# sd-james/gym-treasure-game

Hardware: AMD Instinct MI355X
Metric: env-steps/sec (whole node) at 1M batched envs, 1/2/4/8 MI355X; bit-exact vs CPU (higher is better)
Workload: dtype int32+f64

## Files before the change

gym-treasure-game_amd/_lib.py:

```python
import ctypes
import os

HERE = os.path.dirname(os.path.abspath(__file__))
LIB_PATH = os.environ.get("TG_LIB_PATH") or os.path.join(HERE, "libtg_amd.so")

TG_OK = 0
TG_STEP_AUTORESET = 1
TG_POLICY_UNIFORM = 0
TG_POLICY_MASKED = 1
TG_MODE_DIRECT = 0
TG_MODE_COMPACT = 1
TG_MODE_FLOW = 2
TG_ERR_TICKCAP = 1 << 24
TG_ERR_BAG = 1 << 25
TG_ERR_ACTION = 1 << 26
TG_ERR_NEARINT = 1 << 27
TG_ERR_RENDER = 1 << 28
TG_ERR_WINDOW = 1 << 29
TG_ERR_FLOW = 1 << 30
TG_SPR_COUNT = 24
TG_FRAME_RGB = 3
TG_FRAME_GRAY = 1
TG_ACT_RELU = 0
TG_ACT_TANH = 1
# ... 16 lines not shown

class TgError(RuntimeError):
    pass


class Episode(ctypes.Structure):
    _fields_ = [("env", ctypes.c_int64), ("ret", ctypes.c_int32), ("len", ctypes.c_int32)]


class PyState(ctypes.Structure):
    _fields_ = [("mt", ctypes.c_uint32 * 624), ("index", ctypes.c_uint32),
                ("has_gauss", ctypes.c_uint32), ("gauss_next", ctypes.c_double)]


class Stats(ctypes.Structure):
    _fields_ = [("steps", ctypes.c_int64), ("valid_steps", ctypes.c_int64),
                ("ticks", ctypes.c_int64), ("draws", ctypes.c_int64),
                ("episodes", ctypes.c_int64), ("episodes_dropped", ctypes.c_int64),
                ("launches", ctypes.c_int64),
                ("kernel_ms", ctypes.c_double), ("regens", ctypes.c_int64),
                ("wave_ticks", ctypes.c_int64), ("timed_launches", ctypes.c_int64),
                ("run_ms", ctypes.c_double), ("regen_ms", ctypes.c_double),
                ("regen_timed", ctypes.c_int64), ("regen_launches", ctypes.c_int64),
                ("classify_ms", ctypes.c_double)]

    def as_dict(self):
        return {k: getattr(self, k) for k, _ in self._fields_}


_lib = None


def load():
    global _lib
    if _lib is not None:
        return _lib
    if not os.path.exists(LIB_PATH):
        raise TgError("libtg_amd.so is not built (%s); run __graft_entry__.build() or "
                      "python -m gym_treasure_game_amd.build" % LIB_PATH)
    L = ctypes.CDLL(LIB_PATH)
    P, i32, i64, u32, u64 = (ctypes.c_void_p, ctypes.c_int32, ctypes.c_int64, ctypes.c_uint32,
                             ctypes.c_uint64)
    sig = {
        "tg_create": (i32, [ctypes.POINTER(P), i64, u64, i64, i32, ctypes.c_char_p,
                            ctypes.c_char_p, ctypes.c_char_p]),
        "tg_destroy": (None, [P]),
        "tg_num_envs": (i64, [P]),
# ... 55 lines not shown
```

gym-treasure-game_amd/csrc/tg_amd.hip:

```cpp
#include <hip/hip_runtime.h>

#include <algorithm>
#include <chrono>
#include <cstdio>
#include <cstdlib>
#include <cstring>
#include <mutex>
#include <string>
#include <type_traits>
#include <vector>

#include "../../include/tg_amd.h"
#include "tg_dev.h"
#include "tg_flow.h"
#include "tg_kernels.h"
#include "tg_py1.h"

namespace tg {
thread_local std::string g_err;
}

namespace {

int grid_for(int64_t n) { return (int)((n + BLOCK - 1) / BLOCK); }
int run_grid_for(int64_t n) { return grid_for(n) + (NLIST * 64 + BLOCK - 1) / BLOCK; }
int stat_slots(int64_t n) { return run_grid_for(n); }

#define ALLOC(ptr, bytes)                               \
  if (hipMalloc((void**)&(ptr), (bytes)) != hipSuccess) \
    return fail(TG_E_NOMEM, "hipMalloc %zu B for " #ptr, (size_t)(bytes))

constexpr int KST_MAX = 512;
constexpr int64_t KST_KSLOTS = (int64_t)KST_MAX * 3 * KST_SLOTS;
unsigned long long* kst_step(tg_batch* h, int k, int kernel) {
  return h->kst + ((size_t)k * 2 + kernel) * KST_STRIDE * KST_SLOTS;
}
unsigned long long* kst_regen(tg_batch* h, int k) {
  return h->kst + ((size_t)KST_MAX * 2 + k) * KST_STRIDE * KST_SLOTS;
}
int kst_reset(tg_batch* h) {
  if (!h->kst && hipMalloc((void**)&h->kst, sizeof(unsigned long long) * KST_STRIDE * KST_KSLOTS) !=
                     hipSuccess)
    return fail(TG_E_NOMEM, "timing records");
  hipLaunchKernelGGL(k_kst_init, dim3((unsigned)((KST_KSLOTS + BLOCK - 1) / BLOCK)), dim3(BLOCK), 0, 0,
                     h->kst, KST_KSLOTS);
  HIP_TRY(hipGetLastError());
  HIP_TRY(hipDeviceSynchronize());
  h->kst_steps = 0;
// ... 33 lines not shown
  if (!h->timing_every || (h->timing_calls++ % (uint64_t)h->timing_every) != 0) return TG_OK;
  if (h->kst_steps >= KST_MAX)
    if (const int rc = flush_timing(h)) return rc;
  ks0 = kst_step(h, h->kst_steps, 0);
  ks1 = kst_step(h, h->kst_steps, 1);
  ++h->kst_steps;
  h->kst_k.push_back(k);
  return TG_OK;
}

int alloc_ctx(StepCtx& c, int64_t off, int64_t n) {
  c.off = off;
  c.n = n;
  ALLOC(c.stats, sizeof(unsigned long long) * ST_COUNT * (size_t)stat_slots(n));
  c.shard_cap = (int64_t)((grid_for(n) + WSHARDS - 1) / WSHARDS) * BLOCK;
  ALLOC(c.wl, sizeof(int32_t) * NSEG * (size_t)c.shard_cap);
  ALLOC(c.wst4, sizeof(uint4) * NSEG * (size_t)c.shard_cap);
  ALLOC(c.wang, sizeof(double2) * NSEG * (size_t)c.shard_cap);
  ALLOC(c.wep, sizeof(int2) * NSEG * (size_t)c.shard_cap);
  ALLOC(c.wctr, sizeof(int32_t) * 2 * NCTR * CTR_STRIDE);
  c.rcap = (int64_t)((grid_for(n) + SHARDS - 1) / SHARDS) * BLOCK * REGEN_STEPS;
  ALLOC(c.refill, sizeof(uint32_t) * SHARDS * (size_t)c.rcap);
  ALLOC(c.regen_ctr, sizeof(int32_t) * 2 * RCTR_N * CTR_STRIDE);
  HIP_TRY(hipMemset(c.stats, 0, sizeof(unsigned long long) * ST_COUNT * (size_t)stat_slots(n)));
  HIP_TRY(hipMemset(c.wctr, 0, sizeof(int32_t) * 2 * NCTR * CTR_STRIDE));
  HIP_TRY(hipMemset(c.regen_ctr, 0, sizeof(int32_t) * 2 * RCTR_N * CTR_STRIDE));
  return TG_OK;
}
void free_ctx(StepCtx& c) {
  void* bufs[] = {c.stats, c.wl, c.wst4, c.wang, c.wep, c.wctr, c.refill, c.regen_ctr};
  for (void* b : bufs)
    if (b) (void)hipFree(b);
  if (c.ev) (void)hipEventDestroy(c.ev);
  if (c.st) (void)hipStreamDestroy(c.st);
  c = StepCtx{};
}
Soa soa_of(const tg_batch* h, const StepCtx& c) {
  return Soa{h->S.st4 + c.off, h->S.ang + c.off, h->S.ep + c.off, h->S.mt + c.off * (int64_t)MT_STORE,
             h->S.mc + c.off * (int64_t)MT_CODES};
}
int launch_regen(tg_batch* h, StepCtx& c, hipStream_t st) {
  if (!c.rpend) return TG_OK;
  unsigned long long* ks = nullptr;
  if (h->timing_every && &c == &h->main) {
    if (h->kst_regens >= KST_MAX) {
      const int rc = flush_timing(h);
      if (rc) return rc;
    }
    ks = kst_regen(h, h->kst_regens++);
  }
  if (!h->regen_per_cu) {
    int nb = 0;
    HIP_TRY(hipOccupancyMaxActiveBlocksPerMultiprocessor(&nb, reinterpret_cast<const void*>(k_regen),
// ... 42 lines not shown
    io.valid += c.off;
    io.done += c.off;
    if (io.final_obs) io.final_obs += c.off * 9;
  }
  const bool fo = io.final_obs != nullptr;
  unsigned long long *ks0 = nullptr, *ks1 = nullptr;
  if (&c == &h->main || &c == h->grp.data())
    if (const int rc = timing_begin(h, ks0, ks1)) return rc;
  const EpQueue q{h->eps, h->eps_count, h->eps_cap};
  const dim3 grid(grid_for(c.n)), block(BLOCK);
  const Soa S = soa_of(h, c);
  const int64_t g0 = h->g0 + c.off;
  if (h->mode == TG_MODE_DIRECT) {
    const auto kern = step_inst(ar, fo, io.policy,
                                [](auto AR, auto FO, auto POL) { return &k_step<AR, FO, POL>; });
    hipLaunchKernelGGL(kern, grid, block, 0, st, S, c.n, h->L, h->grid, io, q, g0, c.stats, h->err,
                       ks1);
  } else {
    int32_t* const cur = c.wctr + (c.parity ? NCTR * CTR_STRIDE : 0);
    int32_t* const nxt = c.wctr + (c.parity ? 0 : NCTR * CTR_STRIDE);
    c.parity ^= 1;
    const Work w{c.wl,     c.wst4, c.wang, c.wep, cur, nxt, c.refill,
                 c.regen_ctr + (c.regen_parity * RCTR_N + RCTR_LIST) * CTR_STRIDE, c.rcap,
                 c.shard_cap};
    const auto kc = step_inst(ar, fo, io.policy,
                              [](auto AR, auto FO, auto POL) { return &k_classify<AR, FO, POL>; });
    const auto kr = step_inst(ar, fo, -1, [](auto AR, auto FO, auto) { return &k_run<AR, FO>; });
    hipLaunchKernelGGL(kc, grid, block, 0, st, S, c.n, h->L, h->grid, io, q, w, g0, c.stats, h->err,
                       ks0);
    HIP_TRY(hipGetLastError());
    if (mid) HIP_TRY(hipEventRecord(mid, st));
    hipLaunchKernelGGL(kr, dim3(run_grid_for(c.n) * (BLOCK / RUN_BLOCK)), dim3(RUN_BLOCK), 0, st, S,
                       c.n, h->L, h->grid, io, q, w,
                       g0, c.stats, h->err, ks1);
  }
  HIP_TRY(hipGetLastError());
  if (h->mode != TG_MODE_DIRECT && ++c.rpend == REGEN_STEPS) return launch_regen(h, c, st);
  return TG_OK;
}

int rollout_prep(tg_batch* h, const char* who, int32_t steps, bool selector_ok, const double* obs,
                 const int32_t* reward, const uint8_t* valid, const uint8_t* done) {
  if (steps < 0 || !reward || !valid || !done || !selector_ok)
    return fail(TG_E_INVAL, "%s: bad arguments", who);
  if (!obs && !h->obs_scratch)
    if (hipMalloc((void**)&h->obs_scratch, sizeof(double) * 9 * (size_t)h->n) != hipSuccess)
      return fail(TG_E_NOMEM, "%s: obs scratch", who);
// ... 1015 lines not shown
  HIP_TRY(hipDeviceSynchronize());
  int rc = flush_timing(h);
  if (rc) return rc;
  unsigned long long s[ST_COUNT] = {};
  std::vector<StepCtx*> ctxs{&h->main};
  for (auto& c : h->grp) ctxs.push_back(&c);
  for (StepCtx* c : ctxs) {
    const size_t nb = (size_t)stat_slots(c->n);
    std::vector<unsigned long long> part(nb * ST_COUNT);
    HIP_TRY(hipMemcpy(part.data(), c->stats, sizeof(unsigned long long) * part.size(),
                      hipMemcpyDeviceToHost));
    for (size_t b = 0; b < nb; ++b)
      for (int k = 0; k < ST_COUNT; ++k) s[k] += part[b * ST_COUNT + k];
  }
  out->steps = (int64_t)s[ST_STEPS];
  out->valid_steps = (int64_t)s[ST_VALID];
  out->ticks = (int64_t)s[ST_TICKS];
  out->draws = (int64_t)s[ST_DRAWS];
  out->episodes = (int64_t)s[ST_EPISODES];
  out->episodes_dropped = (int64_t)s[ST_EP_OVERFLOW];
  out->launches = out->steps / (h->n ? h->n : 1);
  out->kernel_ms = h->kernel_ms_done;
  out->regens = (int64_t)s[ST_REGENS] * MT_HALF_GENS;
  out->wave_ticks = (int64_t)s[ST_WTICKS];
  out->timed_launches = h->timed_launches;
  out->run_ms = h->run_ms_done;
  out->regen_ms = h->regen_ms_done;
  out->regen_timed = h->regen_timed;
  out->regen_launches = h->regen_launches;
  out->classify_ms = h->classify_ms_done;
  return TG_OK;
}

int tg_stats_reset(tg_batch* h) {
  BIND(h);
  HIP_TRY(hipDeviceSynchronize());
  HIP_TRY(hipMemset(h->main.stats, 0, sizeof(unsigned long long) * ST_COUNT * (size_t)stat_slots(h->n)));
  for (auto& c : h->grp)
    HIP_TRY(hipMemset(c.stats, 0, sizeof(unsigned long long) * ST_COUNT * (size_t)stat_slots(c.n)));
  if (h->kst) {
    const int rc = kst_reset(h);
    if (rc) return rc;
  }
  h->kernel_ms_done = 0.0;
  h->run_ms_done = 0.0;
  h->classify_ms_done = 0.0;
// ... 65 lines not shown
```

gym-treasure-game_amd/csrc/tg_batch.h:

```cpp
#pragma once
#include <hip/hip_runtime.h>

#include <cstdarg>
#include <cstdio>
#include <string>
#include <vector>

#include "../../include/tg_amd.h"
#include "tg_core.h"

namespace tg {

extern thread_local std::string g_err;
inline int fail(int code, const char* fmt, ...) __attribute__((format(printf, 2, 3)));
inline int fail(int code, const char* fmt, ...) {
  char buf[512];
  va_list ap;
  va_start(ap, fmt);
  vsnprintf(buf, sizeof buf, fmt, ap);
  va_end(ap);
  g_err = buf;
  return code;
}
#define HIP_TRY(expr)                                                                    \
// ... 35 lines not shown
  uint32_t pad2[2];
  uint64_t t_seen, t_end;
  uint32_t ticks;
  uint32_t pad3[7];
  uint64_t phase[5];
  uint64_t pad4[3];
};
static_assert(sizeof(SrvBox) == 192, "SrvBox: three 64-B lines");

struct RenderState;
void render_free(RenderState* rs);

struct StepCtx {
  int64_t off = 0, n = 0;
  unsigned long long* stats = nullptr;
  int32_t* wl = nullptr;
  uint4* wst4 = nullptr;
  double2* wang = nullptr;
  int2* wep = nullptr;
  int32_t* wctr = nullptr;
  uint32_t* refill = nullptr;
  int64_t rcap = 0;
  int64_t shard_cap = 0;
  int parity = 0;
  int rpend = 0;
  int32_t* regen_ctr = nullptr;
  int regen_parity = 0;
  hipStream_t st = nullptr;
  hipEvent_t ev = nullptr;
};

}

struct tg_batch {
  int device = 0;
  int64_t n = 0;
  int64_t g0 = 0;
  uint64_t seed0 = 0;
  tg::Level L{};
  uint32_t* grid = nullptr;
  uint32_t* genrand = nullptr;
  uint32_t* gotab = nullptr;
  uint32_t* masks = nullptr;
  double* obs_q = nullptr;
  int cus = 0;
  tg::Soa S{};
// ... 98 lines not shown
```

gym-treasure-game_amd/csrc/tg_dev.h:

```cpp
#pragma once
#include <hip/hip_runtime.h>

#include "../../include/tg_amd.h"
#include "tg_core.h"
#include "tg_level.h"
#include "tg_batch.h"
#include "tg_twist.h"
#include "tg_run_diag.h"

using namespace tg;

namespace {

constexpr int BLOCK = 256;
#ifndef TG_RUN_BLOCK
#define TG_RUN_BLOCK 256
#endif
constexpr int RUN_BLOCK = TG_RUN_BLOCK;
static_assert(RUN_BLOCK % 64 == 0 && BLOCK % RUN_BLOCK == 0, "whole waves, whole k_classify blocks");
constexpr int PRIO_SLOW = 3;

__device__ __forceinline__ void unpack_st4(const uint4 s, Env& e) {
  e.px = (int)(int16_t)(s.x & 0xFFFFu);
  e.py = (int)(int16_t)(s.x >> 16);
// ... 26 lines not shown
TG_HD int grid_words(int W, int H) { return ((W + 2 * PAD) * (H + 2 * PAD) + 3) / 4; }
template <int NT = BLOCK>
__device__ __forceinline__ void stage_cells(uint32_t* lgrid, uint32_t* ltrig,
                                            const uint32_t* __restrict__ grid, const Level& L,
                                            uint32_t* masks = nullptr) {
  const int nwords = grid_words(L.W, L.H);
  for (int i = threadIdx.x; i < nwords; i += NT) lgrid[i] = grid[i];
  if (threadIdx.x < 12) ltrig[threadIdx.x] = L.trig[threadIdx.x >> 1][threadIdx.x & 1];
  if (masks && L.masks)
    for (int i = threadIdx.x; i < mk_words(L.W, L.H); i += NT) masks[i] = L.masks[i];
  __syncthreads();
}
struct LevelView {
  const uint32_t* trig;
  Map m;
  uint8_t* win;
};
__device__ __forceinline__ LevelView level_in_lds(const uint32_t* __restrict__ grid, const Level& L) {
  __shared__ LdsLevel lv;
  stage_cells(lv.grid, lv.trig, grid, L);
  return {lv.trig, Map{reinterpret_cast<const uint8_t*>(lv.grid), L.W, L.H}, nullptr};
}
template <int NT, int WAVE_BYTES>
__device__ __forceinline__ LevelView run_level_in_lds(const uint32_t* __restrict__ grid, const Level& L) {
  __shared__ uint4 run_lds[((NT / 64) * WAVE_BYTES + MAX_CELLS + 4 * MK_MAX_WORDS) / 16];
  __shared__ uint32_t ltrig[12];
  uint8_t* const win = reinterpret_cast<uint8_t*>(run_lds);
  uint32_t* const lgrid = reinterpret_cast<uint32_t*>(win + (NT / 64) * WAVE_BYTES);
  uint32_t* const lmk = lgrid + grid_words(L.W, L.H);
  stage_cells<NT>(lgrid, ltrig, grid, L, lmk);
  return {ltrig, Map{reinterpret_cast<const uint8_t*>(lgrid), L.W, L.H, L.masks ? lmk : nullptr}, win};
}

__device__ __forceinline__ void store_obs(double* out, int64_t i, const double o[9]) {
  double* p = out + i * 9;
#pragma unroll
  for (int k = 0; k < 9; ++k) p[k] = o[k];
}

constexpr int WIN_UNIT = 16;
constexpr int WIN_DRAWS = 64;
constexpr int WIN_SLOTS = WIN_DRAWS / WIN_UNIT;
constexpr int WIN_SLOT_BYTES = 64 * WIN_UNIT;
constexpr uint32_t CODE_UNITS = MT_CODES / WIN_UNIT;
static_assert(MT_CODES % WIN_UNIT == 0, "whole DMA units of codes per env");
constexpr int WIN_WAVE_BYTES = WIN_SLOTS * WIN_SLOT_BYTES;
constexpr int WAVE_SCRATCH = MT_N * 4;
static_assert(WIN_WAVE_BYTES >= WAVE_SCRATCH, "wave_refill reuses the window as scratch");
static_assert(WIN_DRAWS - WIN_UNIT + 1 >= (int)MAX_TICK_DRAWS, "a refilled window holds a tick's draws");

// ... 251 lines not shown
                                            uint32_t state, lds_u32* scratch) {
  const uint32_t pos = state & MT_POS_MASK;
  const uint32_t dst = (uint32_t)MT_HALF - mt_half(pos);
  const uint64_t src_l = (uint64_t)(uintptr_t)(env_mt + regen_src_off(dst));
  const uint64_t w_l = (uint64_t)(uintptr_t)env_mt;
  const uint64_t c_l = (uint64_t)(uintptr_t)env_mc;
  const int g0_l = (int)(dst / (uint32_t)MT_N);
  while (need) {
    const int L = __ffsll((long long)need) - 1;
    need &= need - 1;
    wave_twist_gens((const glb_u32*)(uintptr_t)readlane64(src_l, L),
                    (glb_u32*)(uintptr_t)readlane64(w_l, L), (uint8_t*)(uintptr_t)readlane64(c_l, L),
                    __builtin_amdgcn_readlane(g0_l, L), MT_HALF_GENS, true, scratch);
  }
}

__device__ __forceinline__ int wave_sum(int v) {
#pragma unroll
  for (int o = 32; o > 0; o >>= 1) v += __shfl_xor(v, o, 64);
  return v;
}

enum { ST_STEPS, ST_VALID, ST_TICKS, ST_DRAWS, ST_EPISODES, ST_EP_OVERFLOW, ST_REGENS, ST_WTICKS,
       ST_COUNT };

__device__ __forceinline__ int wave_max(int v) {
#pragma unroll
  for (int o = 32; o > 0; o >>= 1) v = max(v, __shfl_xor(v, o, 64));
  return v;
}

constexpr int KST_SLOTS = 64;
constexpr int KST_STRIDE = 16;
__device__ __forceinline__ unsigned long long kst_begin(const unsigned long long* ks) {
  return ks ? __builtin_amdgcn_s_memrealtime() : 0ull;
}
__device__ __forceinline__ void kst_end(unsigned long long* ks, unsigned long long t0) {
  if (ks && (threadIdx.x & 63) == 0) {
    unsigned long long* const s = ks + KST_STRIDE * (blockIdx.x % KST_SLOTS);
    atomicMin(s, t0);
    atomicMax(s + 1, (unsigned long long)__builtin_amdgcn_s_memrealtime());
  }
}
struct StepIO {
  int32_t* __restrict__ actions;
  double* __restrict__ obs;
// ... 210 lines not shown
}

constexpr int SHARDS = 8;
#ifndef TG_WSHARDS
#define TG_WSHARDS 8
#endif
constexpr int WSHARDS = TG_WSHARDS;
constexpr int L_RESET = O_COUNT;
constexpr int NLIST = O_COUNT + 1;
struct RunOrder {
  int list[NLIST];
  int seg_base[NLIST];
};
constexpr RunOrder make_run_order() {
  RunOrder r{{O_JUMP_LEFT, O_JUMP_RIGHT, O_GO_LEFT, O_GO_RIGHT, O_DOWN_LEFT, O_DOWN_RIGHT,
              O_UP_LADDER, O_DOWN_LADDER, O_INTERACT, L_RESET},
             {}};
  for (int j = 0; j < NLIST; ++j) r.seg_base[r.list[j]] = j * WSHARDS;
  return r;
}
constexpr RunOrder kRunOrder = make_run_order();
constexpr int NSEG = NLIST * WSHARDS;
static_assert(NSEG <= 2 * RUN_BLOCK, "k_run's prefix: two segments per thread");
constexpr int NCTR = NSEG;
constexpr int CTR_STRIDE = 32;
struct Work {
  int32_t* __restrict__ lists;
  uint4* __restrict__ wst4;
  double2* __restrict__ wang;
  int2* __restrict__ wep;
  int32_t* __restrict__ ctr;
  int32_t* __restrict__ ctr_next;
  uint32_t* __restrict__ refill;
  int32_t* __restrict__ rcnt;
  int64_t rcap;
  int64_t shard_cap;
};
constexpr int REGEN_STEPS = 16;
constexpr int RCTR_LIST = 8;
constexpr int RCTR_N = 16;

struct EnvClass {
  bool runs, rst;
  bool stale;
  int bk;
};
template <bool AUTORESET, int POL>
__device__ __forceinline__ EnvClass classify_env(const Level& L, const Map& m, Env& e, bool live,
                                                 int act, const StepIO& io, int64_t i, int64_t g) {
  EnvClass c{false, false, false, -1};
  int k = -1;
  if (live) {
    if constexpr (POL >= 0) {
      act = policy_action(L, m, e, POL, io.a0, g, io.t);
      if (io.actions) io.actions[i] = act;
    }
    k = option_index(act);
    c.runs = k >= 0 && can_run(L, m, e, k);
    if (k < 0) e.f |= E_ACTION;
  }
  c.rst = AUTORESET && live && !c.runs && is_done(e);
  c.bk = c.runs ? k : c.rst ? L_RESET : -1;
  c.stale = live && (e.mti & (MT_STALE | MT_LISTED)) == MT_STALE;
  if (c.stale) e.mti |= MT_LISTED;
  return c;
}
__device__ __forceinline__ uint32_t refill_entry(int64_t i, uint32_t mti) {
  return (uint32_t)i | (mt_half(mti & MT_POS_MASK) ? 0x80000000u : 0u);
}
template <bool FINAL>
__device__ __forceinline__ void none_rows(const Level& L, const Soa& S, bool fin, Env& e, double2 a2,
                                          int64_t i, int2& ep, const StepIO& io, double* stage,
                                          uint32_t* err_or) {
  double orow[9] = {0, 0, 0, 0, 0, 0, 0, 0, 0};
  if (fin) {
    e.ang0 = a2.x;
    e.ang1 = a2.y;
    Rng rng(S.mt + i * MT_STORE, e.mti, S.mc + i * MT_CODES);
    StepResult r{0, 0, (int)is_done(e), 0};
    finish_step<false, FINAL, false>(L, e, rng, i, r, ep, io, orow);
    if (e.f & E_MASK) atomicOr(err_or, e.f & E_MASK);
  }
  store_obs_wave(io.obs, i - (threadIdx.x & 63), __ballot(fin), orow, stage);
}
struct LaneGroup {
  int rank, lead, nb;
};
__device__ __forceinline__ LaneGroup lane_groups(int bk) {
  LaneGroup g{0, 0, 0};
  unsigned long long pend = __ballot(bk >= 0);
  while (pend) {
// ... 28 lines not shown
```

gym-treasure-game_amd/csrc/tg_kernels.h:

```cpp
#pragma once
#include "tg_dev.h"
#include "tg_flow.h"
#include "tg_policy_mlp.h"

namespace {

__global__ void k_kst_init(unsigned long long* ks, int64_t slots) {
  const int64_t i = (int64_t)blockIdx.x * blockDim.x + threadIdx.x;
  if (i < slots) {
    ks[KST_STRIDE * i] = ~0ull;
    ks[KST_STRIDE * i + 1] = 0ull;
  }
}

__global__ __launch_bounds__(BLOCK) void k_create(Soa S, int64_t n, uint64_t seed0,
                                                   const uint32_t* __restrict__ genrand) {
  const int64_t i = (int64_t)blockIdx.x * BLOCK + threadIdx.x;
  if (i >= n) return;
  seed_mt(S.mt + i * MT_STORE + MT_SEED_OFF, genrand, seed0 + (uint64_t)i);
  Env e{};
  e.mti = 0u;
  S.st4[i] = pack(e);
  S.ang[i] = make_double2(0.0, 0.0);
  S.ep[i] = make_int2(0, 0);
// ... 56 lines not shown
                                                 const uint32_t* __restrict__ grid, StepIO io,
                                                 EpQueue q, int64_t g0,
                                                 unsigned long long* __restrict__ stats,
                                                 uint32_t* __restrict__ err_or,
                                                 unsigned long long* __restrict__ ks) {
  const unsigned long long kt0 = kst_begin(ks);
  __shared__ __attribute__((aligned(16))) uint8_t win[(BLOCK / 64) * WIN_WAVE_BYTES];
  const LevelView lv = level_in_lds(grid, L);
  lds_u8* const wscr = (lds_u8*)win + (threadIdx.x >> 6) * WIN_WAVE_BYTES;
  step_env<AUTORESET, FINAL, POL>(S, n, L, lv.trig, lv.m, wscr, (int64_t)blockIdx.x * BLOCK + threadIdx.x,
                                  io, q, g0, stats, err_or);
  kst_end(ks, kt0);
}

__constant__ RunOrder kRun = kRunOrder;

template <bool AUTORESET, bool FINAL, int POL = -1>
__global__ __launch_bounds__(BLOCK) __attribute__((amdgpu_waves_per_eu(8, 8))) void k_classify(
    Soa S, int64_t n, Level L, const uint32_t* __restrict__ grid, StepIO io, EpQueue q, Work w,
    int64_t g0, unsigned long long* __restrict__ stats, uint32_t* __restrict__ err_or,
    unsigned long long* __restrict__ ks) {
  const unsigned long long kt0 = kst_begin(ks);
  __shared__ int bcnt[NLIST], bbase[NLIST];
  __shared__ int rwc[BLOCK / 64], rbase;
  __shared__ union {
    LdsLevel lv;
    double ostage[BLOCK * 9];
  } lds;
  LdsLevel& lv = lds.lv;
  double* const ostage = lds.ostage;
  const int64_t i = (int64_t)blockIdx.x * BLOCK + threadIdx.x;
  const bool live = i < n;
  const int lane = threadIdx.x & 63;
  uint4 s4 = make_uint4(0, 0, 0, 0);
  int32_t act = 0;
  double2 a2 = make_double2(0.0, 0.0);
  int2 ep = make_int2(0, 0);
  if (live) {
    load_env<false>(S.st4, S.ang, S.ep, i, s4, a2, ep);
    if constexpr (POL < 0) act = io.actions[i];
  }
  if (threadIdx.x < NLIST) bcnt[threadIdx.x] = 0;
  if (blockIdx.x == 0)
    for (int c = threadIdx.x; c < NCTR; c += BLOCK) w.ctr_next[c * CTR_STRIDE] = 0;
  stage_cells(lv.grid, lv.trig, grid, L);
  const Map m{reinterpret_cast<const uint8_t*>(lv.grid), L.W, L.H};
  Env e;
  e.mti = 0u;
  if (live) unpack_st4(s4, e);
  const auto [runs, rst, stale, bk] = classify_env<AUTORESET, POL>(L, m, e, live, act, io, i, g0 + i);
  if (live) io.valid[i] = (uint8_t)runs;
  const unsigned long long sb = __ballot(stale);
  const int srank = __popcll(sb & ((1ull << lane) - 1ull));
  if (lane == 0) rwc[threadIdx.x >> 6] = __popcll(sb);
  const auto [rank, lead, nb] = lane_groups(bk);
  int slot = 0;
  if (bk >= 0 && lane == lead) slot = atomicAdd(&bcnt[bk], nb);
  slot = __shfl(slot, lead, 64) + rank;
  __syncthreads();
  const int shard = blockIdx.x % SHARDS, wshard = blockIdx.x % WSHARDS;
  int my_base = 0;
  if (threadIdx.x < NLIST) {
    const int c = bcnt[threadIdx.x];
    my_base = c ? atomicAdd(&w.ctr[(kRun.seg_base[threadIdx.x] + wshard) * CTR_STRIDE], c) : 0;
  } else if (threadIdx.x == 64) {
    int c = 0;
#pragma unroll
    for (int v = 0; v < BLOCK / 64; ++v) c += rwc[v];
    my_base = c ? atomicAdd(&w.rcnt[shard * CTR_STRIDE], c) : 0;
  }
  const uint4 s4w = pack(e);

  const bool fin = live && !runs && !rst;
  none_rows<FINAL>(L, S, fin, e, a2, i, ep, io, ostage + (threadIdx.x & ~63) * 9, err_or);
  if (fin) {
    const uint4 s4n = pack(e);
    if (s4n.x != s4.x || s4n.y != s4.y || s4n.z != s4.z || s4n.w != s4.w) {
      S.st4[i] = s4n;
    }
  }
  if (threadIdx.x < NLIST) bbase[threadIdx.x] = my_base;
  if (threadIdx.x == 64) rbase = my_base;
  __syncthreads();
  if (stale) {
    int at = rbase + srank;
    for (int v = 0; v < (int)(threadIdx.x >> 6); ++v) at += rwc[v];
    w.refill[shard * w.rcap + at] = refill_entry(i, e.mti);
  }
  if (bk >= 0) {
    const int64_t at = (int64_t)(kRun.seg_base[bk] + wshard) * w.shard_cap + bbase[bk] + slot;
    w.lists[at] = (int32_t)i;
    w.wst4[at] = s4w;
    w.wang[at] = a2;
    w.wep[at] = ep;
  }
  wave_stats(stats, live ? 1 : 0, runs ? 1 : 0, 0, 0, 0);
  kst_end(ks, kt0);
}

template <bool AUTORESET, bool FINAL>
__global__ __launch_bounds__(RUN_BLOCK) void k_run(Soa S, int64_t n, Level L,
                                                const uint32_t* __restrict__ grid, StepIO io,
                                                EpQueue q, Work w, int64_t g0,
                                                unsigned long long* __restrict__ stats,
                                                uint32_t* __restrict__ err_or,
                                                unsigned long long* __restrict__ ks) {
  const unsigned long long kt0 = kst_begin(ks);
  __shared__ int pre[NSEG + 1];
  __shared__ int wtot[RUN_BLOCK / 64];
  __shared__ int ostart[NLIST + 1], oraw[NLIST + 1];
  {
    const int s0 = 2 * (int)threadIdx.x, ln = threadIdx.x & 63;
    const int c0 = s0 < NSEG ? w.ctr[s0 * CTR_STRIDE] : 0;
    const int c1 = s0 + 1 < NSEG ? w.ctr[(s0 + 1) * CTR_STRIDE] : 0;
    int v = c0 + c1;
#pragma unroll
    for (int o = 1; o < 64; o <<= 1) {
      const int y = __shfl_up(v, o, 64);
      if (ln >= o) v += y;
    }
    if (ln == 63) wtot[threadIdx.x >> 6] = v;
    __syncthreads();
    for (int wv = 0; wv < (int)(threadIdx.x >> 6); ++wv) v += wtot[wv];
    const int excl = v - c0 - c1;
    if (s0 < NSEG) pre[s0] = excl;
    if (s0 + 1 < NSEG) pre[s0 + 1] = excl + c0;
    if (threadIdx.x == RUN_BLOCK - 1) pre[NSEG] = v;
  }
  __syncthreads();
  if ((int)(blockIdx.x * RUN_BLOCK) >= pre[NSEG] + NLIST * 63) {
    kst_end(ks, kt0);
    return;
  }
  if (threadIdx.x == 0) {
    int acc = 0;
    for (int j = 0; j < NLIST; ++j) {
      const int sb = j * WSHARDS, se = sb + WSHARDS;
      ostart[j] = acc;
      oraw[j] = pre[sb];
      acc += (pre[se] - pre[sb] + 63) & ~63;
    }
    ostart[NLIST] = acc;
    oraw[NLIST] = pre[NSEG];
  }
  const LevelView lv = run_level_in_lds<RUN_BLOCK, WIN_WAVE_BYTES>(grid, L);
  const int total = ostart[NLIST];
  const int base = (blockIdx.x * RUN_BLOCK + threadIdx.x) & ~63;
  int oj = 0;
  while (oj + 1 < NLIST && ostart[oj + 1] <= base) ++oj;
  oj = __builtin_amdgcn_readfirstlane(oj);
  const int k = kRun.list[oj];
  const int qraw = oraw[oj] + base + (threadIdx.x & 63) - ostart[oj];
  const bool live = base < total && qraw < oraw[oj + 1];
  int seg = oj * WSHARDS;
  if (live) {
    int hi = seg + WSHARDS;
    while (hi - seg > 1) {
      const int mid = (seg + hi) >> 1;
      if (pre[mid] <= qraw) seg = mid; else hi = mid;
    }
  }
  const int idx = qraw - pre[seg];
  int64_t i = 0;
  StepResult r{0, 0, 0, 0};
  Env e;
  e.mti = 0u;
  int2 ep = make_int2(0, 0);
  uint32_t draws = 0;
  int lregen = 0;
  lds_u8* const wscr = (lds_u8*)lv.win + (threadIdx.x >> 6) * WIN_WAVE_BYTES;
  RunStamp stamp;
  stamp.begin();
  if (live) {
    const int64_t at = (int64_t)seg * w.shard_cap + idx;
    i = w.lists[at];
    load_env<false>(w.wst4, w.wang, w.wep, at, e, ep);
    run_listed<AUTORESET, FINAL, false>(L, lv.trig, lv.m, S, i, k, e, ep, wscr, io, err_or, r, draws,
                                        lregen, stamp);
  }
  run_epilogue<AUTORESET, false>(S, live, i, g0 + i, e, ep, nullptr, r, draws, lregen, io.tstep, q, stats,
                                 (int64_t)blockIdx.x / (BLOCK / RUN_BLOCK));
  kst_end(ks, kt0);
  stamp.wave_end(live, k, r.ticks, (int)((blockIdx.x * RUN_BLOCK + threadIdx.x) >> 6));
}

#ifndef TG_REGEN_NT
#define TG_REGEN_NT 0
#endif
constexpr bool REGEN_NT = TG_REGEN_NT != 0;
__global__ __launch_bounds__(BLOCK) void k_regen(Soa S, const uint32_t* __restrict__ refill,
                                                 int64_t rcap, int32_t* __restrict__ ctr,
                                                 int32_t* __restrict__ ctr_next,
                                                 unsigned long long* __restrict__ stats,
                                                 int nstat, unsigned long long* __restrict__ ks) {
  const unsigned long long kt0 = kst_begin(ks);
  __shared__ __attribute__((aligned(16))) uint32_t scratch[BLOCK / 64][MT_N];
  lds_u32* const scr = (lds_u32*)scratch[threadIdx.x >> 6];
  const int lane = threadIdx.x & 63;
  const int xcd = (int)(blockIdx.x & 7u);
  const int64_t cnt = ctr[(RCTR_LIST + xcd) * CTR_STRIDE];
  if (blockIdx.x == 0 && threadIdx.x < RCTR_N) ctr_next[threadIdx.x * CTR_STRIDE] = 0;
  int32_t* const q = ctr + xcd * CTR_STRIDE;
  const uint32_t* const list = refill + xcd * rcap;
  uint32_t* const st_w = reinterpret_cast<uint32_t*>(S.st4);
  auto src_of = [&](uint32_t env, uint32_t s) {
    const uint32_t dst = (uint32_t)MT_HALF - mt_half(s & MT_POS_MASK);
    return (const glb_u32*)(S.mt + (int64_t)env * MT_STORE + regen_src_off(dst));
  };
  const int wx = (int)(blockIdx.x >> 3) * (BLOCK / 64) + (int)(threadIdx.x >> 6);
  const int64_t nwx = (int64_t)((gridDim.x - (unsigned)xcd + 7u) >> 3) * (BLOCK / 64);
  int64_t grab = (cnt + nwx - 1) / nwx;
  if (grab > 64) grab = 64;
  if (grab < 1) grab = 1;
  int halves = 0;
  bool first = true;
  while (true) {
    int64_t j0 = (int64_t)wx * grab;
    if (!first) {
      int g = 0;
      if (lane == 0) g = atomicAdd(q, (int)grab);
      j0 = nwx * grab + __builtin_amdgcn_readfirstlane(g);
    }
    first = false;
    if (j0 >= cnt) break;
    const int64_t m = cnt - j0 < grab ? cnt - j0 : grab;
    const uint32_t env_l = lane < m ? list[j0 + lane] & 0x7FFFFFFFu : 0u;
    const uint32_t st_l = lane < m ? atomicAnd(&st_w[(int64_t)env_l * 4 + 3], ~(MT_STALE | MT_LISTED)) : 0u;
    unsigned long long need = __ballot(lane < m && (st_l & MT_STALE));
    while (need) {
      const int L = __ffsll((long long)need) - 1;
      need &= need - 1;
      const uint32_t env = __builtin_amdgcn_readlane(env_l, L), s = __builtin_amdgcn_readlane(st_l, L);
      const uint32_t dst = (uint32_t)MT_HALF - mt_half(s & MT_POS_MASK);
      TwistIn t;
      twist_load(src_of(env, s), t);
      twist_chain<REGEN_NT>(t, (glb_u32*)(S.mt + (int64_t)env * MT_STORE), S.mc + (int64_t)env * MT_CODES,
                            (int)(dst / (uint32_t)MT_N), MT_HALF_GENS, true, scr);
      ++halves;
    }
  }
  if (lane == 0 && halves)
    atomicAdd(&stats[(size_t)(blockIdx.x % (unsigned)nstat) * ST_COUNT + ST_REGENS],
              (unsigned long long)halves);
  kst_end(ks, kt0);
}

__global__ void k_census(uint32_t* mask) {
  if (threadIdx.x == 0) atomicOr(mask, 1u << (xcc_id() & 31u));
}
__global__ void k_flow_check(const int32_t* __restrict__ ctl, int P, int32_t C,
                             uint32_t* __restrict__ err_or) {
  const int x = (int)threadIdx.x;
  if (x < P) {
    const int Cx = (C - x + P - 1) / P;
    if (Cx > 0 && ctl[(int64_t)x * CTL_WORDS + FC_FIN * FC_STRIDE] != Cx) atomicOr(err_or, E_FLOW);
  }
}

__global__ __launch_bounds__(BLOCK) void k_mask(Soa S, int64_t n, Level L,
                                                 const uint32_t* __restrict__ grid,
                                                 uint16_t* __restrict__ out) {
  const Map m = level_in_lds(grid, L).m;
// ... 137 lines not shown
```

gym-treasure-game_amd/csrc/tg_run_diag.h:

```cpp
#pragma once

namespace {

#ifdef TG_DIAG_STAMPS
constexpr int NSTAMP = 11;
constexpr int NSTAMP_WAVES = 1 << 17;
__device__ unsigned long long g_stamps[NSTAMP_WAVES * NSTAMP];

struct RunPhaseClock {
  unsigned long long ph[4] = {0, 0, 0, 0}, last = 0;
  uint32_t rounds = 0;
  __device__ __forceinline__ void mark(int k) {
    const unsigned long long now = __builtin_amdgcn_s_memtime();
    if (last) ph[k] += now - last;
    last = now;
    rounds += k == 0;
  }
};

struct RunStamp {
  unsigned long long t0 = 0, t1 = 0, t2 = 0, rt0 = 0;
  unsigned long long ph1 = 0, ph2 = 0, ph3 = 0;
  uint32_t rounds = 0;
  __device__ __forceinline__ void begin() {
    t0 = __builtin_amdgcn_s_memtime();
    rt0 = __builtin_amdgcn_s_memrealtime();
  }
  __device__ __forceinline__ void env_loaded() { t1 = __builtin_amdgcn_s_memtime(); }
  __device__ __forceinline__ void option_done(const RunPhaseClock& c) {
    t2 = __builtin_amdgcn_s_memtime();
    ph1 = c.ph[1], ph2 = c.ph[2], ph3 = c.ph[3], rounds = c.rounds;
  }
  __device__ __forceinline__ void wave_end(bool live, int k, int ticks, int wv) const {
    const unsigned long long t3 = __builtin_amdgcn_s_memtime();
    int mx = ticks, sum = ticks;
    for (int o = 32; o > 0; o >>= 1) {
      mx = max(mx, __shfl_xor(mx, o, 64));
      sum += __shfl_xor(sum, o, 64);
    }
    const unsigned long long bl = __ballot(live);
    const int src = bl ? __ffsll((long long)bl) - 1 : 0;
    const unsigned long long a1 = __shfl(t1, src, 64);
    const unsigned long long a2 = __shfl(t2, src, 64);
    const unsigned long long rt3 = __builtin_amdgcn_s_memrealtime();
    int lmax = src;
    unsigned long long best = 0;
    for (int l = 0; l < 64; ++l) {
      const unsigned long long tl = __shfl(ph1 + ph2 + ph3, l, 64);
      if (((bl >> l) & 1ull) && tl > best) best = tl, lmax = l;
    }
    const unsigned long long p1 = __shfl(ph1, lmax, 64), p2 = __shfl(ph2, lmax, 64),
                             p3 = __shfl(ph3, lmax, 64);
    const uint32_t pr = __shfl(rounds, lmax, 64);
    if ((threadIdx.x & 63) == 0 && wv < NSTAMP_WAVES) {
      unsigned long long* const g = g_stamps + (size_t)wv * NSTAMP;
      g[0] = bl ? a1 - t0 : 0;
      g[1] = bl ? a2 - a1 : 0;
      g[2] = bl ? t3 - a2 : t3 - t0;
      g[3] = bl ? (unsigned long long)mx | ((unsigned long long)sum << 32) | ((unsigned long long)k << 56)
                : 1ull | (15ull << 56);
      g[4] = rt0;
      g[5] = rt3;
      g[6] = p1;
      g[7] = p2;
      g[8] = p3;
      g[9] = pr;
      g[10] = 0;
    }
  }
};
#else
struct RunPhaseClock {
  __device__ __forceinline__ void mark(int) {}
};
struct RunStamp {
  __device__ __forceinline__ void begin() {}
  __device__ __forceinline__ void env_loaded() {}
  __device__ __forceinline__ void option_done(const RunPhaseClock&) {}
  __device__ __forceinline__ void wave_end(bool, int, int, int) const {}
};
#endif
struct NoRunHook {
  __device__ __forceinline__ void env_loaded() {}
  __device__ __forceinline__ void option_done(const RunPhaseClock&) {}
};

}
```

include/tg_amd.h:

```cpp
#ifndef TG_AMD_H
#define TG_AMD_H
#include <stdint.h>

#ifdef __cplusplus
extern "C" {
#endif

#define TG_OK 0
#define TG_E_INVAL (-1)
#define TG_E_HIP (-2)
#define TG_E_NOMEM (-3)
#define TG_E_NODEV (-4)
#define TG_E_STATE (-5)

#define TG_OBS_DIM 9
#define TG_NUM_ACTIONS 9

#define TG_ERR_TICKCAP (1u << 24)
#define TG_ERR_BAG (1u << 25)
#define TG_ERR_ACTION (1u << 26)
#define TG_ERR_NEARINT (1u << 27)
#define TG_ERR_RENDER (1u << 28)
#define TG_ERR_WINDOW (1u << 29)
#define TG_ERR_FLOW (1u << 30)
// ... 15 lines not shown
  uint32_t mt[624];
  uint32_t index;
  uint32_t has_gauss;
  double gauss_next;
} tg_pystate;

typedef struct {
  int64_t steps;
  int64_t valid_steps;
  int64_t ticks;
  int64_t draws;
  int64_t episodes;
  int64_t episodes_dropped;
  int64_t launches;
  double kernel_ms;
  int64_t regens;
  int64_t wave_ticks;
  int64_t timed_launches;
  double run_ms;
  double regen_ms;
  int64_t regen_timed;
  int64_t regen_launches;
  double classify_ms;
} tg_stats;

int tg_create(tg_batch **out, int64_t num_envs, uint64_t seed_base, int64_t global_offset,
              int device, const char *domain_txt, const char *objects_txt,
              const char *interactions_txt);
void tg_destroy(tg_batch *h);

int64_t tg_num_envs(const tg_batch *h);

int tg_reset(tg_batch *h, const uint8_t *mask, double *obs, void *stream);

int tg_step(tg_batch *h, const int32_t *actions, double *obs, int32_t *reward, uint8_t *valid,
            uint8_t *done, double *final_obs, uint32_t flags, void *stream);

int tg_step1(tg_batch *h, int32_t action, double *obs, int32_t *reward, uint8_t *valid,
             uint8_t *done, void *stream);

int tg_set_serve(tg_batch *h, int on);

int tg_step1_py(tg_batch *h, int32_t action, tg_pystate *st, double *obs, int32_t *reward,
                uint8_t *valid, uint8_t *done, void *stream);
int tg_reset1_py(tg_batch *h, tg_pystate *st, double *obs, void *stream);

// ... 96 lines not shown
```

Before: 10.29 billion.

## Drain quiet envs' MT regeneration on idle waves of the run kernel

Stale Mersenne-Twister states belonging to envs with no run bucket (quiet) now go into a separate per-shard list instead of the regen kernel's refill list. Waves of k_run that have no chunk to simulate, including trailing blocks past the work, pick up and regenerate these entries at low priority. This hides part of the regen work inside the run kernel's idle tail and shrinks the separate regen launch. In exchange it adds an extra counter, buffer and LDS window setup, and it may lengthen k_run if the idle waves end up doing more work than the tail can hide.

```diff
diff --git a/gym-treasure-game_amd/_lib.py b/gym-treasure-game_amd/_lib.py
--- a/gym-treasure-game_amd/_lib.py
+++ b/gym-treasure-game_amd/_lib.py
@@ -62,7 +62,7 @@
                 ("wave_ticks", ctypes.c_int64), ("timed_launches", ctypes.c_int64),
                 ("run_ms", ctypes.c_double), ("regen_ms", ctypes.c_double),
                 ("regen_timed", ctypes.c_int64), ("regen_launches", ctypes.c_int64),
-                ("classify_ms", ctypes.c_double)]
+                ("classify_ms", ctypes.c_double), ("regens_quiet", ctypes.c_int64)]
 
     def as_dict(self):
         return {k: getattr(self, k) for k, _ in self._fields_}
diff --git a/gym-treasure-game_amd/csrc/tg_amd.hip b/gym-treasure-game_amd/csrc/tg_amd.hip
--- a/gym-treasure-game_amd/csrc/tg_amd.hip
+++ b/gym-treasure-game_amd/csrc/tg_amd.hip
@@ -23,7 +23,7 @@
 namespace {
 
 int grid_for(int64_t n) { return (int)((n + BLOCK - 1) / BLOCK); }
-int run_grid_for(int64_t n) { return grid_for(n) + (NLIST * 64 + BLOCK - 1) / BLOCK; }
+int run_grid_for(int64_t n) { return grid_for(n) + (RUN_EXTRA + BLOCK - 1) / BLOCK; }
 int stat_slots(int64_t n) { return run_grid_for(n); }
 
 #define ALLOC(ptr, bytes)                               \
@@ -103,13 +103,15 @@
   c.rcap = (int64_t)((grid_for(n) + SHARDS - 1) / SHARDS) * BLOCK * REGEN_STEPS;
   ALLOC(c.refill, sizeof(uint32_t) * SHARDS * (size_t)c.rcap);
   ALLOC(c.regen_ctr, sizeof(int32_t) * 2 * RCTR_N * CTR_STRIDE);
+  c.qcap = (int64_t)((grid_for(n) + SHARDS - 1) / SHARDS) * BLOCK;
+  ALLOC(c.quiet, sizeof(uint32_t) * SHARDS * (size_t)c.qcap);
   HIP_TRY(hipMemset(c.stats, 0, sizeof(unsigned long long) * ST_COUNT * (size_t)stat_slots(n)));
   HIP_TRY(hipMemset(c.wctr, 0, sizeof(int32_t) * 2 * NCTR * CTR_STRIDE));
   HIP_TRY(hipMemset(c.regen_ctr, 0, sizeof(int32_t) * 2 * RCTR_N * CTR_STRIDE));
   return TG_OK;
 }
 void free_ctx(StepCtx& c) {
-  void* bufs[] = {c.stats, c.wl, c.wst4, c.wang, c.wep, c.wctr, c.refill, c.regen_ctr};
+  void* bufs[] = {c.stats, c.wl, c.wst4, c.wang, c.wep, c.wctr, c.refill, c.regen_ctr, c.quiet};
   for (void* b : bufs)
     if (b) (void)hipFree(b);
   if (c.ev) (void)hipEventDestroy(c.ev);
@@ -198,7 +200,7 @@
     c.parity ^= 1;
     const Work w{c.wl,     c.wst4, c.wang, c.wep, cur, nxt, c.refill,
                  c.regen_ctr + (c.regen_parity * RCTR_N + RCTR_LIST) * CTR_STRIDE, c.rcap,
-                 c.shard_cap};
+                 c.shard_cap, c.quiet, c.qcap};
     const auto kc = step_inst(ar, fo, io.policy,
                               [](auto AR, auto FO, auto POL) { return &k_classify<AR, FO, POL>; });
     const auto kr = step_inst(ar, fo, -1, [](auto AR, auto FO, auto) { return &k_run<AR, FO>; });
@@ -1260,6 +1262,7 @@
   out->launches = out->steps / (h->n ? h->n : 1);
   out->kernel_ms = h->kernel_ms_done;
   out->regens = (int64_t)s[ST_REGENS] * MT_HALF_GENS;
+  out->regens_quiet = (int64_t)s[ST_RQUIET] * MT_HALF_GENS;
   out->wave_ticks = (int64_t)s[ST_WTICKS];
   out->timed_launches = h->timed_launches;
   out->run_ms = h->run_ms_done;
diff --git a/gym-treasure-game_amd/csrc/tg_batch.h b/gym-treasure-game_amd/csrc/tg_batch.h
--- a/gym-treasure-game_amd/csrc/tg_batch.h
+++ b/gym-treasure-game_amd/csrc/tg_batch.h
@@ -81,6 +81,8 @@
   uint32_t* refill = nullptr;
   int64_t rcap = 0;
   int64_t shard_cap = 0;
+  uint32_t* quiet = nullptr;
+  int64_t qcap = 0;
   int parity = 0;
   int rpend = 0;
   int32_t* regen_ctr = nullptr;
diff --git a/gym-treasure-game_amd/csrc/tg_dev.h b/gym-treasure-game_amd/csrc/tg_dev.h
--- a/gym-treasure-game_amd/csrc/tg_dev.h
+++ b/gym-treasure-game_amd/csrc/tg_dev.h
@@ -72,10 +72,14 @@
   return {lv.trig, Map{reinterpret_cast<const uint8_t*>(lv.grid), L.W, L.H}, nullptr};
 }
 template <int NT, int WAVE_BYTES>
+__device__ __forceinline__ uint8_t* run_lds_win() {
+  __shared__ uint4 run_lds[((NT / 64) * WAVE_BYTES + MAX_CELLS + 4 * MK_MAX_WORDS) / 16];
+  return reinterpret_cast<uint8_t*>(run_lds);
+}
+template <int NT, int WAVE_BYTES>
 __device__ __forceinline__ LevelView run_level_in_lds(const uint32_t* __restrict__ grid, const Level& L) {
-  __shared__ uint4 run_lds[((NT / 64) * WAVE_BYTES + MAX_CELLS + 4 * MK_MAX_WORDS) / 16];
   __shared__ uint32_t ltrig[12];
-  uint8_t* const win = reinterpret_cast<uint8_t*>(run_lds);
+  uint8_t* const win = run_lds_win<NT, WAVE_BYTES>();
   uint32_t* const lgrid = reinterpret_cast<uint32_t*>(win + (NT / 64) * WAVE_BYTES);
   uint32_t* const lmk = lgrid + grid_words(L.W, L.H);
   stage_cells<NT>(lgrid, ltrig, grid, L, lmk);
@@ -373,6 +377,7 @@
 }
 
 enum { ST_STEPS, ST_VALID, ST_TICKS, ST_DRAWS, ST_EPISODES, ST_EP_OVERFLOW, ST_REGENS, ST_WTICKS,
+       ST_RQUIET,
        ST_COUNT };
 
 __device__ __forceinline__ int wave_max(int v) {
@@ -629,8 +634,12 @@
 constexpr RunOrder kRunOrder = make_run_order();
 constexpr int NSEG = NLIST * WSHARDS;
 static_assert(NSEG <= 2 * RUN_BLOCK, "k_run's prefix: two segments per thread");
-constexpr int NCTR = NSEG;
+constexpr int QCTR = NSEG;
+constexpr int NCTR = NSEG + SHARDS;
 constexpr int CTR_STRIDE = 32;
+constexpr int RUN_EXTRA = NLIST * 64;
+static_assert(RUN_EXTRA > NLIST * 63 && BLOCK % 64 == 0 && RUN_BLOCK % 64 == 0,
+              "a k_run grid always has a wave without a chunk");
 struct Work {
   int32_t* __restrict__ lists;
   uint4* __restrict__ wst4;
@@ -642,6 +651,8 @@
   int32_t* __restrict__ rcnt;
   int64_t rcap;
   int64_t shard_cap;
+  uint32_t* __restrict__ quiet;
+  int64_t qcap;
 };
 constexpr int REGEN_STEPS = 16;
 constexpr int RCTR_LIST = 8;
@@ -674,6 +685,26 @@
 }
 __device__ __forceinline__ uint32_t refill_entry(int64_t i, uint32_t mti) {
   return (uint32_t)i | (mt_half(mti & MT_POS_MASK) ? 0x80000000u : 0u);
+}
+template <bool NT>
+__device__ __forceinline__ int regen_entries(const Soa& S, bool mine, uint32_t env_l, lds_u32* scr) {
+  uint32_t* const st_w = reinterpret_cast<uint32_t*>(S.st4);
+  const uint32_t st_l = mine ? atomicAnd(&st_w[(int64_t)env_l * 4 + 3], ~(MT_STALE | MT_LISTED)) : 0u;
+  unsigned long long need = __ballot(mine && (st_l & MT_STALE));
+  int halves = 0;
+  while (need) {
+    const int L = __ffsll((long long)need) - 1;
+    need &= need - 1;
+    const uint32_t env = __builtin_amdgcn_readlane(env_l, L), s = __builtin_amdgcn_readlane(st_l, L);
+    const uint32_t dst = (uint32_t)MT_HALF - mt_half(s & MT_POS_MASK);
+    uint32_t* const mt = S.mt + (int64_t)env * MT_STORE;
+    TwistIn t;
+    twist_load((const glb_u32*)(mt + regen_src_off(dst)), t);
+    twist_chain<NT>(t, (glb_u32*)mt, S.mc + (int64_t)env * MT_CODES, (int)(dst / (uint32_t)MT_N),
+                    MT_HALF_GENS, true, scr);
+    ++halves;
+  }
+  return halves;
 }
 template <bool FINAL>
 __device__ __forceinline__ void none_rows(const Level& L, const Soa& S, bool fin, Env& e, double2 a2,
diff --git a/gym-treasure-game_amd/csrc/tg_kernels.h b/gym-treasure-game_amd/csrc/tg_kernels.h
--- a/gym-treasure-game_amd/csrc/tg_kernels.h
+++ b/gym-treasure-game_amd/csrc/tg_kernels.h
@@ -102,7 +102,7 @@
     unsigned long long* __restrict__ ks) {
   const unsigned long long kt0 = kst_begin(ks);
   __shared__ int bcnt[NLIST], bbase[NLIST];
-  __shared__ int rwc[BLOCK / 64], rbase;
+  __shared__ int rwc[BLOCK / 64], rbase, qwc[BLOCK / 64], qbase;
   __shared__ union {
     LdsLevel lv;
     double ostage[BLOCK * 9];
@@ -130,9 +130,13 @@
   if (live) unpack_st4(s4, e);
   const auto [runs, rst, stale, bk] = classify_env<AUTORESET, POL>(L, m, e, live, act, io, i, g0 + i);
   if (live) io.valid[i] = (uint8_t)runs;
-  const unsigned long long sb = __ballot(stale);
-  const int srank = __popcll(sb & ((1ull << lane) - 1ull));
-  if (lane == 0) rwc[threadIdx.x >> 6] = __popcll(sb);
+  const bool quiet = bk < 0;
+  const unsigned long long qb = __ballot(stale && quiet), db = __ballot(stale && !quiet);
+  const int srank = __popcll((quiet ? qb : db) & ((1ull << lane) - 1ull));
+  if (lane == 0) {
+    rwc[threadIdx.x >> 6] = __popcll(db);
+    qwc[threadIdx.x >> 6] = __popcll(qb);
+  }
   const auto [rank, lead, nb] = lane_groups(bk);
   int slot = 0;
   if (bk >= 0 && lane == lead) slot = atomicAdd(&bcnt[bk], nb);
@@ -148,6 +152,11 @@
 #pragma unroll
     for (int v = 0; v < BLOCK / 64; ++v) c += rwc[v];
     my_base = c ? atomicAdd(&w.rcnt[shard * CTR_STRIDE], c) : 0;
+  } else if (threadIdx.x == 128) {
+    int c = 0;
+#pragma unroll
+    for (int v = 0; v < BLOCK / 64; ++v) c += qwc[v];
+    my_base = c ? atomicAdd(&w.ctr[(QCTR + shard) * CTR_STRIDE], c) : 0;
   }
   const uint4 s4w = pack(e);
 
@@ -161,11 +170,12 @@
   }
   if (threadIdx.x < NLIST) bbase[threadIdx.x] = my_base;
   if (threadIdx.x == 64) rbase = my_base;
+  if (threadIdx.x == 128) qbase = my_base;
   __syncthreads();
   if (stale) {
-    int at = rbase + srank;
-    for (int v = 0; v < (int)(threadIdx.x >> 6); ++v) at += rwc[v];
-    w.refill[shard * w.rcap + at] = refill_entry(i, e.mti);
+    int at = (quiet ? qbase : rbase) + srank;
+    for (int v = 0; v < (int)(threadIdx.x >> 6); ++v) at += quiet ? qwc[v] : rwc[v];
+    (quiet ? w.quiet + shard * w.qcap : w.refill + shard * w.rcap)[at] = refill_entry(i, e.mti);
   }
   if (bk >= 0) {
     const int64_t at = (int64_t)(kRun.seg_base[bk] + wshard) * w.shard_cap + bbase[bk] + slot;
@@ -176,6 +186,43 @@
   }
   wave_stats(stats, live ? 1 : 0, runs ? 1 : 0, 0, 0, 0);
   kst_end(ks, kt0);
+}
+
+__device__ __forceinline__ int quiet_drain(const Soa& S, const Work& w, const int* pre, int base,
+                                           lds_u32* scr, unsigned long long* __restrict__ stats) {
+  __builtin_amdgcn_s_setprio(0);
+  int qp[SHARDS + 1];
+  qp[0] = 0;
+#pragma unroll
+  for (int x = 0; x < SHARDS; ++x) qp[x + 1] = qp[x] + w.ctr[(QCTR + x) * CTR_STRIDE];
+  const int64_t tot = qp[SHARDS];
+  if (!tot) return 0;
+  int total = 0;
+  for (int j = 0; j < NLIST; ++j) total += (pre[(j + 1) * WSHARDS] - pre[j * WSHARDS] + 63) & ~63;
+  const int64_t nidle = (int64_t)gridDim.x * (RUN_BLOCK / 64) - (total >> 6);
+  int64_t grab = (tot + nidle - 1) / nidle;
+  if (grab > 64) grab = 64;
+  const int lane = threadIdx.x & 63;
+  int halves = 0;
+  for (int64_t j0 = (int64_t)((base - total) >> 6) * grab; j0 < tot; j0 += nidle * grab) {
+    const int64_t j = j0 + lane;
+    const bool mine = lane < grab && j < tot;
+    uint32_t env_l = 0u;
+    if (mine) {
+      int x = 0, lo = 0;
+#pragma unroll
+      for (int y = 1; y < SHARDS; ++y)
+        if (j >= qp[y]) x = y, lo = qp[y];
+      env_l = w.quiet[x * w.qcap + (j - lo)] & 0x7FFFFFFFu;
+    }
+    halves += regen_entries<false>(S, mine, env_l, scr);
+  }
+  if (lane == 0 && halves) {
+    unsigned long long* const slot = stats + (size_t)(blockIdx.x / (BLOCK / RUN_BLOCK)) * ST_COUNT;
+    atomicAdd(&slot[ST_REGENS], (unsigned long long)halves);
+    atomicAdd(&slot[ST_RQUIET], (unsigned long long)halves);
+  }
+  return halves;
 }
 
 template <bool AUTORESET, bool FINAL>
@@ -208,24 +255,33 @@
     if (threadIdx.x == RUN_BLOCK - 1) pre[NSEG] = v;
   }
   __syncthreads();
-  if ((int)(blockIdx.x * RUN_BLOCK) >= pre[NSEG] + NLIST * 63) {
+  const int base = (blockIdx.x * RUN_BLOCK + threadIdx.x) & ~63;
+  const bool past = (int)(blockIdx.x * RUN_BLOCK) >= pre[NSEG] + NLIST * 63;
+  LevelView lv{nullptr, Map{nullptr, 0, 0}, run_lds_win<RUN_BLOCK, WIN_WAVE_BYTES>()};
+  if (!past) {
+    if (threadIdx.x == 0) {
+      int acc = 0;
+      for (int j = 0; j < NLIST; ++j) {
+        const int sb = j * WSHARDS, se = sb + WSHARDS;
+        ostart[j] = acc;
+        oraw[j] = pre[sb];
+        acc += (pre[se] - pre[sb] + 63) & ~63;
+      }
+      ostart[NLIST] = acc;
+      oraw[NLIST] = pre[NSEG];
+    }
+    lv = run_level_in_lds<RUN_BLOCK, WIN_WAVE_BYTES>(grid, L);
+  }
+  lds_u8* const wscr = (lds_u8*)lv.win + (threadIdx.x >> 6) * WIN_WAVE_BYTES;
+  RunStamp stamp;
+  stamp.begin();
+  if (past || base >= ostart[NLIST]) {
+    const int halves = quiet_drain(S, w, pre, base, (lds_u32*)wscr, stats);
     kst_end(ks, kt0);
+    stamp.wave_end(false, 0, 0, base >> 6, halves);
     return;
   }
-  if (threadIdx.x == 0) {
-    int acc = 0;
-    for (int j = 0; j < NLIST; ++j) {
-      const int sb = j * WSHARDS, se = sb + WSHARDS;
-      ostart[j] = acc;
-      oraw[j] = pre[sb];
-      acc += (pre[se] - pre[sb] + 63) & ~63;
-    }
-    ostart[NLIST] = acc;
-    oraw[NLIST] = pre[NSEG];
-  }
-  const LevelView lv = run_level_in_lds<RUN_BLOCK, WIN_WAVE_BYTES>(grid, L);
   const int total = ostart[NLIST];
-  const int base = (blockIdx.x * RUN_BLOCK + threadIdx.x) & ~63;
   int oj = 0;
   while (oj + 1 < NLIST && ostart[oj + 1] <= base) ++oj;
   oj = __builtin_amdgcn_readfirstlane(oj);
@@ -248,9 +304,6 @@
   int2 ep = make_int2(0, 0);
   uint32_t draws = 0;
   int lregen = 0;
-  lds_u8* const wscr = (lds_u8*)lv.win + (threadIdx.x >> 6) * WIN_WAVE_BYTES;
-  RunStamp stamp;
-  stamp.begin();
   if (live) {
     const int64_t at = (int64_t)seg * w.shard_cap + idx;
     i = w.lists[at];
@@ -261,7 +314,7 @@
   run_epilogue<AUTORESET, false>(S, live, i, g0 + i, e, ep, nullptr, r, draws, lregen, io.tstep, q, stats,
                                  (int64_t)blockIdx.x / (BLOCK / RUN_BLOCK));
   kst_end(ks, kt0);
-  stamp.wave_end(live, k, r.ticks, (int)((blockIdx.x * RUN_BLOCK + threadIdx.x) >> 6));
+  stamp.wave_end(live, k, r.ticks, base >> 6);
 }
 
 #ifndef TG_REGEN_NT
@@ -282,11 +335,6 @@
   if (blockIdx.x == 0 && threadIdx.x < RCTR_N) ctr_next[threadIdx.x * CTR_STRIDE] = 0;
   int32_t* const q = ctr + xcd * CTR_STRIDE;
   const uint32_t* const list = refill + xcd * rcap;
-  uint32_t* const st_w = reinterpret_cast<uint32_t*>(S.st4);
-  auto src_of = [&](uint32_t env, uint32_t s) {
-    const uint32_t dst = (uint32_t)MT_HALF - mt_half(s & MT_POS_MASK);
-    return (const glb_u32*)(S.mt + (int64_t)env * MT_STORE + regen_src_off(dst));
-  };
   const int wx = (int)(blockIdx.x >> 3) * (BLOCK / 64) + (int)(threadIdx.x >> 6);
   const int64_t nwx = (int64_t)((gridDim.x - (unsigned)xcd + 7u) >> 3) * (BLOCK / 64);
   int64_t grab = (cnt + nwx - 1) / nwx;
@@ -305,19 +353,7 @@
     if (j0 >= cnt) break;
     const int64_t m = cnt - j0 < grab ? cnt - j0 : grab;
     const uint32_t env_l = lane < m ? list[j0 + lane] & 0x7FFFFFFFu : 0u;
-    const uint32_t st_l = lane < m ? atomicAnd(&st_w[(int64_t)env_l * 4 + 3], ~(MT_STALE | MT_LISTED)) : 0u;
-    unsigned long long need = __ballot(lane < m && (st_l & MT_STALE));
-    while (need) {
-      const int L = __ffsll((long long)need) - 1;
-      need &= need - 1;
-      const uint32_t env = __builtin_amdgcn_readlane(env_l, L), s = __builtin_amdgcn_readlane(st_l, L);
-      const uint32_t dst = (uint32_t)MT_HALF - mt_half(s & MT_POS_MASK);
-      TwistIn t;
-      twist_load(src_of(env, s), t);
-      twist_chain<REGEN_NT>(t, (glb_u32*)(S.mt + (int64_t)env * MT_STORE), S.mc + (int64_t)env * MT_CODES,
-                            (int)(dst / (uint32_t)MT_N), MT_HALF_GENS, true, scr);
-      ++halves;
-    }
+    halves += regen_entries<REGEN_NT>(S, lane < m, env_l, scr);
   }
   if (lane == 0 && halves)
     atomicAdd(&stats[(size_t)(blockIdx.x % (unsigned)nstat) * ST_COUNT + ST_REGENS],
diff --git a/gym-treasure-game_amd/csrc/tg_run_diag.h b/gym-treasure-game_amd/csrc/tg_run_diag.h
--- a/gym-treasure-game_amd/csrc/tg_run_diag.h
+++ b/gym-treasure-game_amd/csrc/tg_run_diag.h
@@ -31,7 +31,7 @@
     t2 = __builtin_amdgcn_s_memtime();
     ph1 = c.ph[1], ph2 = c.ph[2], ph3 = c.ph[3], rounds = c.rounds;
   }
-  __device__ __forceinline__ void wave_end(bool live, int k, int ticks, int wv) const {
+  __device__ __forceinline__ void wave_end(bool live, int k, int ticks, int wv, int halves = 0) const {
     const unsigned long long t3 = __builtin_amdgcn_s_memtime();
     int mx = ticks, sum = ticks;
     for (int o = 32; o > 0; o >>= 1) {
@@ -65,7 +65,7 @@
       g[7] = p2;
       g[8] = p3;
       g[9] = pr;
-      g[10] = 0;
+      g[10] = (unsigned long long)halves;
     }
   }
 };
@@ -77,7 +77,7 @@
   __device__ __forceinline__ void begin() {}
   __device__ __forceinline__ void env_loaded() {}
   __device__ __forceinline__ void option_done(const RunPhaseClock&) {}
-  __device__ __forceinline__ void wave_end(bool, int, int, int) const {}
+  __device__ __forceinline__ void wave_end(bool, int, int, int, int = 0) const {}
 };
 #endif
 struct NoRunHook {
diff --git a/include/tg_amd.h b/include/tg_amd.h
--- a/include/tg_amd.h
+++ b/include/tg_amd.h
@@ -61,6 +61,7 @@
   int64_t regen_timed;
   int64_t regen_launches;
   double classify_ms;
+  int64_t regens_quiet;
 } tg_stats;
 
 int tg_create(tg_batch **out, int64_t num_envs, uint64_t seed_base, int64_t global_offset,
```

New measurement: 11.11 billion (median of 6 runs). 8.0% higher.
